# UM-ARM-Lab/pytorch_volumetric

Hardware: AMD Instinct MI355X
Metric: SDF (val+grad) queries/sec (higher is better)
Workload: dtype f32

## Files before the change

pytorch_volumetric_amd/csrc/cached.hip:

```cpp
#include "common.h"
#include "grid_lookup.h"

namespace pvamd {

constexpr int kWavesPerBlock = 16;
constexpr int kTilePoints = 256;
constexpr int64_t kWaveTileMinPoints = 16384;
constexpr int kCqMinWaves = 1;
constexpr int64_t kCqStreamFrom = (int64_t)8 << 20;
constexpr bool kCqBigStNt = true, kCqBigLdNt = true;
constexpr int64_t kCqBlocks = 1024, kCqBigBlocks = 0;

template <bool F64, bool WRITE_OOB, bool LD_NT, bool ST_NT>
__global__ __launch_bounds__(kWavesPerBlock * 64, kCqMinWaves) void cached_query_wave(const pvamd_grid_t g,
                                                                         const float* __restrict__ pts, int64_t P,
                                                                         float* __restrict__ val,
                                                                         float* __restrict__ grad,
                                                                         uint8_t* __restrict__ oob) {
    __shared__ __attribute__((aligned(16))) float lds[kWavesPerBlock][1024];
    const int lane = threadIdx.x & 63, wave = threadIdx.x >> 6;
    float* spf = lds[wave];
    f32x4_alias* sp = reinterpret_cast<f32x4_alias*>(spf);
    const int64_t ntiles = (P + kTilePoints - 1) / kTilePoints;
    const int64_t wstride = (int64_t)gridDim.x * kWavesPerBlock;
    int64_t tile = (int64_t)blockIdx.x * kWavesPerBlock + wave;
    auto first_point = [&](int64_t t) { return t * kTilePoints <= P - kTilePoints ? t * kTilePoints : P - kTilePoints; };
    f32x4 a, b, c;
    auto load3 = [&](int64_t t) {
        const f32x4_u* src = reinterpret_cast<const f32x4_u*>(pts + 3 * first_point(t));
        if (LD_NT) {
            a = __builtin_nontemporal_load(src + lane);
            b = __builtin_nontemporal_load(src + lane + 64);
            c = __builtin_nontemporal_load(src + lane + 128);
        } else {
            a = src[lane];
            b = src[lane + 64];
            c = src[lane + 128];
        }
    };
    if (tile < ntiles) load3(tile);
    for (; tile < ntiles; tile += wstride) {
        sp[lane] = a;
        sp[lane + 64] = b;
        sp[lane + 128] = c;
        const int64_t next = tile + wstride;
        if (next < ntiles) load3(next);
        PVAMD_WAVE_SYNC();
        float px[4], py[4], pz[4];
        const f32x4 q0 = sp[3 * lane], q1 = sp[3 * lane + 1], q2 = sp[3 * lane + 2];
        px[0] = q0.x; py[0] = q0.y; pz[0] = q0.z;
        px[1] = q0.w; py[1] = q1.x; pz[1] = q1.y;
        px[2] = q1.z; py[2] = q1.w; pz[2] = q2.x;
        px[3] = q2.y; py[3] = q2.z; pz[3] = q2.w;
        PVAMD_WAVE_SYNC();
        const int64_t o = first_point(tile);
        float4 r[4];
        bool valid[4];
#pragma unroll
        for (int k = 0; k < 4; ++k) {
            r[k] = cached_lookup<F64, LD_NT>(g, px[k], py[k], pz[k], valid[k]);
        }
        sp[3 * lane] = f32x4{r[0].y, r[0].z, r[0].w, r[1].y};
        sp[3 * lane + 1] = f32x4{r[1].z, r[1].w, r[2].y, r[2].z};
        sp[3 * lane + 2] = f32x4{r[2].w, r[3].y, r[3].z, r[3].w};
        const f32x4 v4 = f32x4{r[0].x, r[1].x, r[2].x, r[3].x};
        if constexpr (WRITE_OOB) {
            const uint32_t m = (valid[0] ? 0u : 1u) | (valid[1] ? 0u : 1u << 8) | (valid[2] ? 0u : 1u << 16) | (valid[3] ? 0u : 1u << 24);
            __builtin_memcpy(oob + o + 4 * lane, &m, 4);
        }
        PVAMD_WAVE_SYNC();
        f32x4_u* vdst = reinterpret_cast<f32x4_u*>(val + o);
        f32x4_u* dst = reinterpret_cast<f32x4_u*>(grad + 3 * o);
        if (ST_NT) {
            __builtin_nontemporal_store(v4, vdst + lane);
            __builtin_nontemporal_store(sp[lane], dst + lane);
            __builtin_nontemporal_store(sp[lane + 64], dst + lane + 64);
            __builtin_nontemporal_store(sp[lane + 128], dst + lane + 128);
        } else {
            vdst[lane] = v4;
            dst[lane] = sp[lane];
            dst[lane + 64] = sp[lane + 64];
            dst[lane + 128] = sp[lane + 128];
        }
        PVAMD_WAVE_SYNC();
    }
}

template <bool F64, bool WRITE_OOB, int PPL, int WAVES>
__global__ __launch_bounds__(WAVES * 64) void cached_query_direct(const pvamd_grid_t g, const float* __restrict__ pts, int64_t P,
                                                                  float* __restrict__ val, float* __restrict__ grad,
                                                                  uint8_t* __restrict__ oob) {
    constexpr int kTile = 64 * PPL;
    const int lane = threadIdx.x & 63, wave = threadIdx.x >> 6;
    const int64_t tile = (int64_t)blockIdx.x * WAVES + wave;
    if (tile * kTile >= P) return;
    const int64_t o = (tile * kTile <= P - kTile ? tile * kTile : P - kTile) + lane;
    float px[PPL], py[PPL], pz[PPL];
#pragma unroll
    for (int k = 0; k < PPL; ++k) {
        const int64_t i = o + 64 * k;
        px[k] = pts[3 * i];
        py[k] = pts[3 * i + 1];
        pz[k] = pts[3 * i + 2];
    }
#pragma unroll
    for (int k = 0; k < PPL; ++k) {
        const int64_t i = o + 64 * k;
        bool valid;
        const float4 r = cached_lookup<F64, false>(g, px[k], py[k], pz[k], valid);
        __builtin_nontemporal_store(r.x, val + i);
        __builtin_nontemporal_store(r.y, grad + 3 * i);
        __builtin_nontemporal_store(r.z, grad + 3 * i + 1);
        __builtin_nontemporal_store(r.w, grad + 3 * i + 2);
        if constexpr (WRITE_OOB) oob[i] = valid ? 0 : 1;
    }
}

enum CqKind {
    kCqScalar = PVAMD_CQ_KERNEL_SCALAR, kCqDirect1 = PVAMD_CQ_KERNEL_DIRECT_1, kCqDirect2 = PVAMD_CQ_KERNEL_DIRECT_2,
    kCqDirect2Wide = PVAMD_CQ_KERNEL_DIRECT_2W, kCqDirect4 = PVAMD_CQ_KERNEL_DIRECT_4, kCqWaveTile = PVAMD_CQ_KERNEL_WAVE_TILE,
    kCqStreaming = PVAMD_CQ_KERNEL_STREAMING
};
static inline CqKind cq_kind(int64_t P) {
    if (P < kWaveTileMinPoints) return kCqScalar;
    if (P <= 160 * 1024) return kCqDirect1;
    if (P <= 896 * 1024) return kCqDirect2;
    if (P <= 1024 * 1024) return kCqDirect2Wide;
    if (P <= 1600 * 1024) return kCqDirect4;
    if (P <= 2304 * 1024) return kCqWaveTile;
    if (P <= kCqStreamFrom) return kCqDirect4;
    return kCqStreaming;
}

template <bool F64>
__global__ __launch_bounds__(256) void cached_query_scalar(const pvamd_grid_t g, const float* __restrict__ pts,
                                                            int64_t first, int64_t P, float* __restrict__ val,
                                                            float* __restrict__ grad, uint8_t* __restrict__ oob) {
    const int64_t stride = (int64_t)gridDim.x * blockDim.x;
    for (int64_t i = first + (int64_t)blockIdx.x * blockDim.x + threadIdx.x; i < P; i += stride) {
        bool valid;
        const float4 r = cached_lookup<F64>(g, pts[3 * i], pts[3 * i + 1], pts[3 * i + 2], valid);
        val[i] = r.x;
        grad[3 * i] = r.y;
        grad[3 * i + 1] = r.z;
        grad[3 * i + 2] = r.w;
        if (oob) oob[i] = valid ? 0 : 1;
    }
}

template <bool F64>
__global__ __launch_bounds__(256) void cached_outside_kernel(const pvamd_grid_t g, const float* __restrict__ pts,
                                                              int64_t P, float level, uint8_t* __restrict__ out) {
    const int64_t stride = (int64_t)gridDim.x * blockDim.x;
    for (int64_t i = (int64_t)blockIdx.x * blockDim.x + threadIdx.x; i < P; i += stride) {
        int flat;
        const bool valid = voxel_flat<F64>(g, pts[3 * i], pts[3 * i + 1], pts[3 * i + 2], flat);
        out[i] = valid ? (uint8_t)(g.vox[4 * (int64_t)flat] > level) : (uint8_t)1;
    }
}

template <bool F64>
__global__ __launch_bounds__(256) void voxel_index_kernel(const pvamd_grid_t g, const float* __restrict__ pts,
                                                           int64_t P, int64_t* __restrict__ out_key,
                                                           int64_t* __restrict__ out_flat,
                                                           uint8_t* __restrict__ out_valid) {
    const int64_t stride = (int64_t)gridDim.x * blockDim.x;
    for (int64_t i = (int64_t)blockIdx.x * blockDim.x + threadIdx.x; i < P; i += stride) {
        long long key[3];
        const bool valid = voxel_key<F64>(g, pts[3 * i], pts[3 * i + 1], pts[3 * i + 2], key);
        if (out_key) {
            out_key[3 * i] = key[0];
            out_key[3 * i + 1] = key[1];
            out_key[3 * i + 2] = key[2];
        }
        if (out_flat) out_flat[i] = (key[0] * g.shape[1] + key[1]) * g.shape[2] + key[2];
        if (out_valid) out_valid[i] = valid ? 1 : 0;
    }
}

__global__ __launch_bounds__(256) void cached_outside_f64_kernel(const pvamd_grid_t g, const double* __restrict__ pts,
                                                                  int64_t P, double level, uint8_t* __restrict__ out) {
    const int64_t stride = (int64_t)gridDim.x * blockDim.x;
    for (int64_t i = (int64_t)blockIdx.x * blockDim.x + threadIdx.x; i < P; i += stride) {
        const double p[3] = {pts[3 * i], pts[3 * i + 1], pts[3 * i + 2]};
        long long key[3];
        const bool valid = voxel_key_f64(g, p, key);
        out[i] = valid ? (uint8_t)(g.vox[4 * (int64_t)clamped_flat(g, key)] > (float)level) : (uint8_t)1;
    }
}

__global__ __launch_bounds__(256) void voxel_index_f64_kernel(const pvamd_grid_t g, const double* __restrict__ pts,
                                                               int64_t P, int64_t* __restrict__ out_key,
                                                               int64_t* __restrict__ out_flat,
                                                               uint8_t* __restrict__ out_valid) {
    const int64_t stride = (int64_t)gridDim.x * blockDim.x;
    for (int64_t i = (int64_t)blockIdx.x * blockDim.x + threadIdx.x; i < P; i += stride) {
        const double p[3] = {pts[3 * i], pts[3 * i + 1], pts[3 * i + 2]};
        long long key[3];
        const bool valid = voxel_key_f64(g, p, key);
        if (out_key) {
            out_key[3 * i] = key[0];
            out_key[3 * i + 1] = key[1];
            out_key[3 * i + 2] = key[2];
        }
        if (out_flat) out_flat[i] = (key[0] * g.shape[1] + key[1]) * g.shape[2] + key[2];
        if (out_valid) out_valid[i] = valid ? 1 : 0;
    }
}

__global__ __launch_bounds__(256) void pack_grid_kernel(const float* __restrict__ val, const float* __restrict__ grad,
                                                         int64_t n, float4* __restrict__ out) {
    const int64_t stride = (int64_t)gridDim.x * blockDim.x;
    for (int64_t i = (int64_t)blockIdx.x * blockDim.x + threadIdx.x; i < n; i += stride) {
        out[i] = make_float4(val[i], grad[3 * i], grad[3 * i + 1], grad[3 * i + 2]);
    }
}

}

using namespace pvamd;

extern "C" int pvamd_pack_grid(const float* val, const float* grad, int64_t n, float* out, void* stream) {
    if (!val || !grad || !out) return PVAMD_E_NULL;
    if (n < 0) return PVAMD_E_SHAPE;
    if (!aligned_to(out, 16)) return PVAMD_E_ALIGN;
    if (n == 0) return 0;
    hipLaunchKernelGGL(pack_grid_kernel, dim3(stream_grid(n, 256)), dim3(256), 0, (hipStream_t)stream, val, grad, n,
                       reinterpret_cast<float4*>(out));
    return (int)hipGetLastError();
}

extern "C" int pvamd_cached_query_kernel(int64_t P) { return (int)cq_kind(P); }

extern "C" int pvamd_cached_query(const pvamd_grid_t* grid, const float* points, int64_t P, float* out_val,
                                  float* out_grad, uint8_t* out_oob, void* stream) {
    if (P < 0) return PVAMD_E_SHAPE;
    if (P == 0) return 0;
    if (!grid || !out_val || !out_grad || !points) return PVAMD_E_NULL;
    if (int e = check_grid(*grid)) return e;
    if (!aligned_to(points, 4) || !aligned_to(out_val, 4) || !aligned_to(out_grad, 4)) return PVAMD_E_ALIGN;
    hipStream_t s = (hipStream_t)stream;
    const bool f64 = grid->index_f64 != 0;
    const CqKind kind = cq_kind(P);
    if (kind == kCqWaveTile || kind == kCqStreaming) {
        const int64_t ntiles = (P + kTilePoints - 1) / kTilePoints;
        const int64_t need = (ntiles + kWavesPerBlock - 1) / kWavesPerBlock;
        const bool big = kind == kCqStreaming;
        const int64_t cap = big ? kCqBigBlocks : kCqBlocks;
        const dim3 grid_dim((unsigned)((cap > 0 && need > cap) ? cap : need)), block(kWavesPerBlock * 64);
#define PVAMD_LAUNCH_CQ(F64_, OOB_)                                                                                      \
    do {                                                                                                                \
        if (big) hipLaunchKernelGGL((cached_query_wave<F64_, OOB_, kCqBigLdNt, kCqBigStNt>), grid_dim, block, 0, s, *grid, points, P, out_val, out_grad, out_oob); \
        else hipLaunchKernelGGL((cached_query_wave<F64_, OOB_, false, true>), grid_dim, block, 0, s, *grid, points, P, out_val, out_grad, out_oob);    \
    } while (0)
        if (f64) {
            if (out_oob) PVAMD_LAUNCH_CQ(true, true);
            else PVAMD_LAUNCH_CQ(true, false);
        } else {
            if (out_oob) PVAMD_LAUNCH_CQ(false, true);
            else PVAMD_LAUNCH_CQ(false, false);
        }
#undef PVAMD_LAUNCH_CQ
    } else if (kind != kCqScalar) {
#define PVAMD_LAUNCH_DIRECT(PPL_, WAVES_)                                                                               \
    do {                                                                                                                \
        const int64_t tiles_ = (P + 64 * PPL_ - 1) / (64 * PPL_);                                                       \
        const dim3 grid_dim((unsigned)((tiles_ + WAVES_ - 1) / WAVES_)), block(WAVES_ * 64);                            \
        if (f64) {                                                                                                      \
            if (out_oob) hipLaunchKernelGGL((cached_query_direct<true, true, PPL_, WAVES_>), grid_dim, block, 0, s, *grid, points, P, out_val, out_grad, out_oob);   \
            else hipLaunchKernelGGL((cached_query_direct<true, false, PPL_, WAVES_>), grid_dim, block, 0, s, *grid, points, P, out_val, out_grad, out_oob);        \
        } else {                                                                                                        \
            if (out_oob) hipLaunchKernelGGL((cached_query_direct<false, true, PPL_, WAVES_>), grid_dim, block, 0, s, *grid, points, P, out_val, out_grad, out_oob);  \
            else hipLaunchKernelGGL((cached_query_direct<false, false, PPL_, WAVES_>), grid_dim, block, 0, s, *grid, points, P, out_val, out_grad, out_oob);       \
        }                                                                                                               \
    } while (0)
        if (kind == kCqDirect1) PVAMD_LAUNCH_DIRECT(1, 8);
        else if (kind == kCqDirect2) PVAMD_LAUNCH_DIRECT(2, 4);
        else if (kind == kCqDirect2Wide) PVAMD_LAUNCH_DIRECT(2, 16);
        else PVAMD_LAUNCH_DIRECT(4, 4);
#undef PVAMD_LAUNCH_DIRECT
    } else {
        const dim3 grid_dim(stream_grid(P, 256)), block(256);
        if (f64) hipLaunchKernelGGL((cached_query_scalar<true>), grid_dim, block, 0, s, *grid, points, (int64_t)0, P, out_val, out_grad, out_oob);
        else hipLaunchKernelGGL((cached_query_scalar<false>), grid_dim, block, 0, s, *grid, points, (int64_t)0, P, out_val, out_grad, out_oob);
    }
    return (int)hipGetLastError();
}

extern "C" int pvamd_cached_outside(const pvamd_grid_t* grid, const float* points, int64_t P, float level,
                                    uint8_t* out, void* stream) {
    if (P < 0) return PVAMD_E_SHAPE;
    if (P == 0) return 0;
    if (!grid || !out || !points) return PVAMD_E_NULL;
    if (int e = check_grid(*grid)) return e;
    const dim3 grid_dim(stream_grid(P, 256)), block(256);
    if (grid->index_f64) hipLaunchKernelGGL((cached_outside_kernel<true>), grid_dim, block, 0, (hipStream_t)stream, *grid, points, P, level, out);
    else hipLaunchKernelGGL((cached_outside_kernel<false>), grid_dim, block, 0, (hipStream_t)stream, *grid, points, P, level, out);
    return (int)hipGetLastError();
}

extern "C" int pvamd_voxel_index(const pvamd_grid_t* grid, const float* points, int64_t P, int64_t* out_key,
                                 int64_t* out_flat, uint8_t* out_valid, void* stream) {
    if (P < 0) return PVAMD_E_SHAPE;
    if (P == 0) return 0;
    if (!grid || !points) return PVAMD_E_NULL;
    if (int e = check_grid(*grid, false)) return e;
    const dim3 grid_dim(stream_grid(P, 256)), block(256);
    if (grid->index_f64) hipLaunchKernelGGL((voxel_index_kernel<true>), grid_dim, block, 0, (hipStream_t)stream, *grid, points, P, out_key, out_flat, out_valid);
    else hipLaunchKernelGGL((voxel_index_kernel<false>), grid_dim, block, 0, (hipStream_t)stream, *grid, points, P, out_key, out_flat, out_valid);
    return (int)hipGetLastError();
}

extern "C" int pvamd_cached_outside_f64(const pvamd_grid_t* grid, const double* points, int64_t P, double level,
                                        uint8_t* out, void* stream) {
    if (P < 0) return PVAMD_E_SHAPE;
    if (P == 0) return 0;
    if (!grid || !out || !points) return PVAMD_E_NULL;
    if (int e = check_grid(*grid)) return e;
    if (!aligned_to(points, 8)) return PVAMD_E_ALIGN;
    hipLaunchKernelGGL(cached_outside_f64_kernel, dim3(stream_grid(P, 256)), dim3(256), 0, (hipStream_t)stream, *grid,
                       points, P, level, out);
    return (int)hipGetLastError();
}

extern "C" int pvamd_voxel_index_f64(const pvamd_grid_t* grid, const double* points, int64_t P, int64_t* out_key,
                                     int64_t* out_flat, uint8_t* out_valid, void* stream) {
    if (P < 0) return PVAMD_E_SHAPE;
    if (P == 0) return 0;
    if (!grid || !points) return PVAMD_E_NULL;
    if (int e = check_grid(*grid, false)) return e;
    if (!aligned_to(points, 8)) return PVAMD_E_ALIGN;
    hipLaunchKernelGGL(voxel_index_f64_kernel, dim3(stream_grid(P, 256)), dim3(256), 0, (hipStream_t)stream, *grid, points,
                       P, out_key, out_flat, out_valid);
    return (int)hipGetLastError();
}
```

pytorch_volumetric_amd/csrc/grid_lookup.h:

```cpp
#pragma once
#include <hip/hip_runtime.h>
#include <stdint.h>
#include "exact_math.h"
#include "../../include/pvamd.h"

namespace pvamd {

#define PVAMD_DEV __device__ __forceinline__

typedef float record_f32x4 __attribute__((ext_vector_type(4)));
typedef const record_f32x4 __attribute__((address_space(1))) * global_record_ptr;
PVAMD_DEV float4 load_record(const float* vox, int flat) {
    const record_f32x4 r = ((global_record_ptr)(uintptr_t)vox)[flat];
    return make_float4(r.x, r.y, r.z, r.w);
}

template <typename T>
PVAMD_DEV T round_by_rule(int rule, T q) {
    if (rule & PVAMD_RULE_ROUND_HALF_AWAY) {
        if constexpr (sizeof(T) == 8) return __builtin_round(q);
        else return __builtin_roundf(q);
    }
    if (rule & PVAMD_RULE_ROUND_FLOOR_HALF) {
        if constexpr (sizeof(T) == 8) return __builtin_floor(q + 0.5);
        else return __builtin_floorf(add_rn(q, 0.5f));
    }
    if constexpr (sizeof(T) == 8) return __builtin_rint(q);
    else return __builtin_rintf(q);
}

PVAMD_DEV bool voxel_index_1d_ruled(const pvamd_grid_t& g, int d, float p, bool f64, long long& k) {
    double kq;
    if (f64) kq = round_by_rule<double>(g.rule, ((double)p - g.dmin[d]) / g.dres[d]);
    else kq = (double)round_by_rule<float>(g.rule, div_rn(sub_rn(p, g.fmin[d]), g.fres[d]));
    k = (long long)kq;
    if (g.rule & PVAMD_RULE_VALID_ON_INDEX) return (kq >= 0.0) && (kq <= (double)(g.shape[d] - 1));
    return f64 ? (g.dmin[d] <= (double)p) && ((double)p <= g.dmax[d]) : (g.fmin[d] <= p) && (p <= g.fmax[d]);
}

template <bool F64>
PVAMD_DEV bool voxel_index_1d(const pvamd_grid_t& g, int d, float p, long long& k) {
    if (__builtin_expect(g.rule != 0, 0)) return voxel_index_1d_ruled(g, d, p, F64, k);
    if constexpr (F64) {
        const double pd = (double)p;
        const bool valid = (g.dmin[d] <= pd) && (pd <= g.dmax[d]);
        k = (long long)__builtin_rint((pd - g.dmin[d]) / g.dres[d]);
        return valid;
    } else {
        const bool valid = (g.fmin[d] <= p) && (p <= g.fmax[d]);
        k = (long long)__builtin_rintf(div_rn(sub_rn(p, g.fmin[d]), g.fres[d]));
        return valid;
    }
}

template <bool F64>
PVAMD_DEV bool voxel_key(const pvamd_grid_t& g, float x, float y, float z, long long key[3]) {
    const bool vx = voxel_index_1d<F64>(g, 0, x, key[0]);
    const bool vy = voxel_index_1d<F64>(g, 1, y, key[1]);
    const bool vz = voxel_index_1d<F64>(g, 2, z, key[2]);
    return vx & vy & vz;
}

template <bool F64>
PVAMD_DEV bool voxel_flat(const pvamd_grid_t& g, float x, float y, float z, int& flat) {
    long long key[3];
    const bool valid = voxel_key<F64>(g, x, y, z, key);
    int kx = (int)key[0], ky = (int)key[1], kz = (int)key[2];
    kx = min(max(kx, 0), g.shape[0] - 1);
    ky = min(max(ky, 0), g.shape[1] - 1);
    kz = min(max(kz, 0), g.shape[2] - 1);
    flat = (kx * g.shape[1] + ky) * g.shape[2] + kz;
    return valid;
}

PVAMD_DEV bool in_range(const pvamd_grid_t& g, float x, float y, float z) {
    return (g.vlo[0] <= x) & (x <= g.vhi[0]) & (g.vlo[1] <= y) & (y <= g.vhi[1]) & (g.vlo[2] <= z) & (z <= g.vhi[2]);
}

PVAMD_DEV uint64_t in_range_mask(const pvamd_grid_t& g, float x, float y, float z) {
    return __builtin_amdgcn_ballot_w64(__builtin_amdgcn_fmed3f(x, g.vlo[0], g.vhi[0]) == x) &
           __builtin_amdgcn_ballot_w64(__builtin_amdgcn_fmed3f(y, g.vlo[1], g.vhi[1]) == y) &
           __builtin_amdgcn_ballot_w64(__builtin_amdgcn_fmed3f(z, g.vlo[2], g.vhi[2]) == z);
}

template <bool F64>
PVAMD_DEV int voxel_index_fast(const pvamd_grid_t& g, int d, float p) {
    const float t = mul_rn(sub_rn(p, g.fmin[d]), g.inv32[d]);
    const float kc = __builtin_rintf(t);
    const float half_dist = sub_rn(0.5f, fabsf(sub_rn(t, kc)));
    if (half_dist > g.err32[d]) return (int)kc;
    long long k;
    voxel_index_1d<F64>(g, d, p, k);
    return (int)k;
}

PVAMD_DEV bool wave_all(bool p) { return __builtin_amdgcn_ballot_w64(p) == __builtin_amdgcn_ballot_w64(true); }
PVAMD_DEV bool wave_any(bool p) { return __builtin_amdgcn_ballot_w64(p) != 0; }

PVAMD_DEV float sqrt_rn_sumsq(float n2) {
    const bool tiny = (unsigned)(__float_as_int(n2) - 1) < (unsigned)(0x0F800000 - 1);
    if (__builtin_expect(wave_any(tiny), 0)) return sqrt_rn(n2);
    float s = __builtin_amdgcn_sqrtf(n2);
    const float s_dn = __int_as_float(__float_as_int(s) - 1), s_up = __int_as_float(__float_as_int(s) + 1);
    const float r_dn = fmaf(-s_dn, s, n2), r_up = fmaf(-s_up, s, n2);
    s = (r_dn <= 0.f) ? s_dn : s;
    s = (r_up > 0.f) ? s_up : s;
    return s;
}

PVAMD_DEV bool estimate_unsure(const pvamd_grid_t& g, const float off[3]) {
    const float worst = __builtin_fmaxf(__builtin_fmaxf(fabsf(off[0]), fabsf(off[1])), fabsf(off[2]));
    return !(sub_rn(0.5f, worst) > g.err32[0]);
}

PVAMD_DEV int voxel_flat_estimate(const pvamd_grid_t& g, float x, float y, float z, bool& unsure) {
    const float p[3] = {x, y, z};
    int k[3];
    float off[3];
#pragma unroll
    for (int d = 0; d < 3; ++d) {
        const float t = mul_rn(sub_rn(p[d], g.fmin[d]), g.inv32[d]);
        const float kc = __builtin_rintf(t);
        off[d] = sub_rn(t, kc);
        k[d] = (int)kc;
    }
    unsure |= estimate_unsure(g, off);
    const unsigned flat = (unsigned)((k[0] * g.shape[1] + k[1]) * g.shape[2] + k[2]);
    const unsigned last = (unsigned)(g.shape[0] * g.shape[1] * g.shape[2] - 1);
    return (int)(flat < last ? flat : last);
}

PVAMD_DEV int voxel_flat_in_range_fused(const pvamd_grid_t& g, float x, float y, float z) {
    const float p[3] = {x, y, z};
    int k[3];
    float off[3];
#pragma unroll
    for (int d = 0; d < 3; ++d) {
        const float t = mul_rn(sub_rn(p[d], g.fmin[d]), g.inv32[d]);
        const float kc = __builtin_rintf(t);
        off[d] = sub_rn(t, kc);
        k[d] = (int)kc;
    }
    const bool unsure = estimate_unsure(g, off);
    if (__builtin_expect(wave_any(unsure), 0)) {
        if (unsure) {
#pragma unroll 1
            for (int d = 0; d < 3; ++d) {
                long long kd;
                if (g.index_f64) voxel_index_1d<true>(g, d, p[d], kd);
                else voxel_index_1d<false>(g, d, p[d], kd);
                k[d] = (int)kd;
            }
        }
    }
    const unsigned flat = (unsigned)((k[0] * g.shape[1] + k[1]) * g.shape[2] + k[2]);
    const unsigned last = (unsigned)(g.shape[0] * g.shape[1] * g.shape[2] - 1);
    return (int)(flat < last ? flat : last);
}

template <bool F64>
PVAMD_DEV int voxel_flat_in_range(const pvamd_grid_t& g, float x, float y, float z) {
    int kx = voxel_index_fast<F64>(g, 0, x), ky = voxel_index_fast<F64>(g, 1, y), kz = voxel_index_fast<F64>(g, 2, z);
    kx = min(max(kx, 0), g.shape[0] - 1);
    ky = min(max(ky, 0), g.shape[1] - 1);
    kz = min(max(kz, 0), g.shape[2] - 1);
    return (kx * g.shape[1] + ky) * g.shape[2] + kz;
}

PVAMD_DEV float bounding_box_vector(const pvamd_grid_t& g, float x, float y, float z, float t[3]) {
    const float p[3] = {x, y, z};
#pragma unroll
    for (int d = 0; d < 3; ++d) {
        float lo = sub_rn(g.bb_min[d], p[d]);
        const bool lo_active = lo > 0.f;
        lo = lo_active ? lo : 0.f;
        float hi = sub_rn(p[d], g.bb_max[d]);
        hi = (hi > 0.f) ? hi : 0.f;
        const float s = add_rn(lo, hi);
        t[d] = lo_active ? -s : s;
    }
    return sqrt_rn(fmaf(t[2], t[2], fmaf(t[1], t[1], mul_rn(t[0], t[0]))));
}

PVAMD_DEV float4 bounding_box_sdf(const pvamd_grid_t& g, float x, float y, float z) {
    float t[3];
    const float n = bounding_box_vector(g, x, y, z, t);
    return make_float4(n, div_rn(t[0], n), div_rn(t[1], n), div_rn(t[2], n));
}

template <bool F64, bool STREAMING = false>
PVAMD_DEV float4 cached_lookup(const pvamd_grid_t& g, float x, float y, float z, bool& valid) {
    if constexpr (STREAMING) {
        valid = in_range(g, x, y, z);
        if (valid) {
            return reinterpret_cast<const float4*>(g.vox)[voxel_flat_in_range<F64>(g, x, y, z)];
        }
        if (g.oob_mode == PVAMD_OOB_BOUNDING_BOX) {
            return bounding_box_sdf(g, x, y, z);
        }
        return make_float4(0.f, 0.f, 0.f, 0.f);
    } else {
        valid = (__builtin_amdgcn_fmed3f(x, g.vlo[0], g.vhi[0]) == x) & (__builtin_amdgcn_fmed3f(y, g.vlo[1], g.vhi[1]) == y) &
                (__builtin_amdgcn_fmed3f(z, g.vlo[2], g.vhi[2]) == z);
        if (valid) return reinterpret_cast<const float4*>(g.vox)[voxel_flat_in_range_fused(g, x, y, z)];
        if (g.oob_mode == PVAMD_OOB_BOUNDING_BOX) {
            const float ta = __builtin_amdgcn_fmed3f(sub_rn(x, g.bb_min[0]), sub_rn(x, g.bb_max[0]), 0.f);
            const float tb = __builtin_amdgcn_fmed3f(sub_rn(y, g.bb_min[1]), sub_rn(y, g.bb_max[1]), 0.f);
            const float tc = __builtin_amdgcn_fmed3f(sub_rn(z, g.bb_min[2]), sub_rn(z, g.bb_max[2]), 0.f);
            const float n = sqrt_rn_sumsq(fmaf(tc, tc, fmaf(tb, tb, mul_rn(ta, ta))));
            return make_float4(n, div_rn(ta, n), div_rn(tb, n), div_rn(tc, n));
        }
        return make_float4(0.f, 0.f, 0.f, 0.f);
    }
}

PVAMD_DEV bool voxel_key_f64(const pvamd_grid_t& g, const double p[3], long long key[3]) {
    bool valid = true;
#pragma unroll
    for (int d = 0; d < 3; ++d) {
        const double kq = round_by_rule<double>(g.rule, (p[d] - g.dmin[d]) / g.dres[d]);
        key[d] = (long long)kq;
        if (__builtin_expect(g.rule & PVAMD_RULE_VALID_ON_INDEX, 0)) valid &= (kq >= 0.0) && (kq <= (double)(g.shape[d] - 1));
        else valid &= (g.dmin[d] <= p[d]) && (p[d] <= g.dmax[d]);
    }
    return valid;
}

PVAMD_DEV int clamped_flat(const pvamd_grid_t& g, const long long key[3]) {
    const int kx = min(max((int)key[0], 0), g.shape[0] - 1);
    const int ky = min(max((int)key[1], 0), g.shape[1] - 1);
    const int kz = min(max((int)key[2], 0), g.shape[2] - 1);
    return (kx * g.shape[1] + ky) * g.shape[2] + kz;
}

PVAMD_DEV float affine_row(float m0, float m1, float m2, float m3, float px, float py, float pz) {
    return add_rn(fmaf(m2, pz, fmaf(m1, py, mul_rn(m0, px))), m3);
}

template <typename T> struct LeafOps;

template <> struct LeafOps<float> {
    static PVAMD_DEV void xform(const float* M, const float p[3], float x[3]) {
        x[0] = affine_row(M[0], M[1], M[2], M[3], p[0], p[1], p[2]);
        x[1] = affine_row(M[4], M[5], M[6], M[7], p[0], p[1], p[2]);
        x[2] = affine_row(M[8], M[9], M[10], M[11], p[0], p[1], p[2]);
    }
    static PVAMD_DEV bool inside(const pvamd_grid_t& g, const float x[3]) { return in_range(g, x[0], x[1], x[2]); }
    static PVAMD_DEV void record_grad(const pvamd_grid_t& g, const float x[3], float gr[3]) {
        int flat;
        if (g.index_f64) voxel_flat<true>(g, x[0], x[1], x[2], flat);
        else voxel_flat<false>(g, x[0], x[1], x[2], flat);
        const float4 r = load_record(g.vox, flat);
        gr[0] = r.y; gr[1] = r.z; gr[2] = r.w;
    }
    static PVAMD_DEV float box(const pvamd_grid_t& g, const float x[3], float t[3]) {
        return bounding_box_vector(g, x[0], x[1], x[2], t);
    }
    static PVAMD_DEV float div(float a, float b) { return div_rn(a, b); }
};

template <> struct LeafOps<double> {
    static PVAMD_DEV void xform(const double* M, const double p[3], double x[3]) {
#pragma unroll
        for (int r = 0; r < 3; ++r)
            x[r] = __builtin_fma(M[4 * r + 2], p[2], __builtin_fma(M[4 * r + 1], p[1], M[4 * r] * p[0])) + M[4 * r + 3];
    }
    static PVAMD_DEV bool inside(const pvamd_grid_t& g, const double x[3]) {
        long long key[3];
        return voxel_key_f64(g, x, key);
    }
    static PVAMD_DEV void record_grad(const pvamd_grid_t& g, const double x[3], double gr[3]) {
        long long key[3];
        voxel_key_f64(g, x, key);
        const float4 r = load_record(g.vox, clamped_flat(g, key));
        gr[0] = (double)r.y; gr[1] = (double)r.z; gr[2] = (double)r.w;
    }
    static PVAMD_DEV double box(const pvamd_grid_t& g, const double x[3], double t[3]) {
#pragma unroll
        for (int d = 0; d < 3; ++d) {
            double lo = g.dbb_min[d] - x[d];
            const bool lo_active = lo > 0.0;
            lo = lo_active ? lo : 0.0;
            double hi = x[d] - g.dbb_max[d];
            hi = (hi > 0.0) ? hi : 0.0;
            const double s = lo + hi;
            t[d] = lo_active ? -s : s;
        }
        return __builtin_sqrt(__builtin_fma(t[2], t[2], __builtin_fma(t[1], t[1], t[0] * t[0])));
    }
    static PVAMD_DEV double div(double a, double b) { return a / b; }
};

}
```

Baseline: 203.0 billion.

## Batch voxel record gathers in direct kernel and compute bbox fallback branch-free

The direct cached-query kernel now computes validity and flat indices for all PPL points per lane first, with a wave-uniform slow path for uncertain indices. It then issues all record loads back to back, computes the bounding-box fallback unconditionally, and selects results per point. This is meant to expose memory-level parallelism across the gathered loads instead of serialising lookup, load and store per point, at the cost of extra ALU work and registers for the unconditional bbox math. The early return for out-of-range tiles is removed, and the wave-tile size threshold is lowered slightly.

```diff
diff --git a/pytorch_volumetric_amd/csrc/cached.hip b/pytorch_volumetric_amd/csrc/cached.hip
--- a/pytorch_volumetric_amd/csrc/cached.hip
+++ b/pytorch_volumetric_amd/csrc/cached.hip
@@ -90,10 +90,10 @@
 __global__ __launch_bounds__(WAVES * 64) void cached_query_direct(const pvamd_grid_t g, const float* __restrict__ pts, int64_t P,
                                                                   float* __restrict__ val, float* __restrict__ grad,
                                                                   uint8_t* __restrict__ oob) {
+    static_assert(PPL >= 1 && PPL <= 4, "the gathered records live in four named variables");
     constexpr int kTile = 64 * PPL;
     const int lane = threadIdx.x & 63, wave = threadIdx.x >> 6;
     const int64_t tile = (int64_t)blockIdx.x * WAVES + wave;
-    if (tile * kTile >= P) return;
     const int64_t o = (tile * kTile <= P - kTile ? tile * kTile : P - kTile) + lane;
     float px[PPL], py[PPL], pz[PPL];
 #pragma unroll
@@ -103,16 +103,48 @@
         py[k] = pts[3 * i + 1];
         pz[k] = pts[3 * i + 2];
     }
+    bool valid[PPL], unsure[PPL];
+    int flat[PPL];
+    bool any_unsure = false;
+#pragma unroll
+    for (int k = 0; k < PPL; ++k) {
+        valid[k] = in_range_med3(g, px[k], py[k], pz[k]);
+        unsure[k] = false;
+        flat[k] = voxel_flat_estimate(g, px[k], py[k], pz[k], unsure[k]);
+        unsure[k] &= valid[k];
+        any_unsure |= unsure[k];
+    }
+    if (__builtin_expect(wave_any(any_unsure), 0)) {
+#pragma unroll
+        for (int k = 0; k < PPL; ++k) {
+            if (unsure[k]) voxel_flat<F64>(g, px[k], py[k], pz[k], flat[k]);
+        }
+    }
+    record_f32x4 rec_a, rec_b, rec_c, rec_d;
+    if (valid[0]) rec_a = load_record_bits(g.vox, flat[0]);
+    if constexpr (PPL > 1) { if (valid[1]) rec_b = load_record_bits(g.vox, flat[1]); }
+    if constexpr (PPL > 2) { if (valid[2]) rec_c = load_record_bits(g.vox, flat[2]); }
+    if constexpr (PPL > 3) { if (valid[3]) rec_d = load_record_bits(g.vox, flat[3]); }
+    const bool bbox = g.oob_mode == PVAMD_OOB_BOUNDING_BOX;
+    float4 ob[PPL];
+#pragma unroll
+    for (int k = 0; k < PPL; ++k) {
+        ob[k] = bbox ? bounding_box_record(g, px[k], py[k], pz[k]) : make_float4(0.f, 0.f, 0.f, 0.f);
+    }
 #pragma unroll
     for (int k = 0; k < PPL; ++k) {
         const int64_t i = o + 64 * k;
-        bool valid;
-        const float4 r = cached_lookup<F64, false>(g, px[k], py[k], pz[k], valid);
-        __builtin_nontemporal_store(r.x, val + i);
-        __builtin_nontemporal_store(r.y, grad + 3 * i);
-        __builtin_nontemporal_store(r.z, grad + 3 * i + 1);
-        __builtin_nontemporal_store(r.w, grad + 3 * i + 2);
-        if constexpr (WRITE_OOB) oob[i] = valid ? 0 : 1;
+        const bool v = valid[k];
+        const record_f32x4& rec = k == 0 ? rec_a : k == 1 ? rec_b : k == 2 ? rec_c : rec_d;
+        const uint32_t r0 = v ? __float_as_uint(rec.x) : __float_as_uint(ob[k].x);
+        const uint32_t r1 = v ? __float_as_uint(rec.y) : __float_as_uint(ob[k].y);
+        const uint32_t r2 = v ? __float_as_uint(rec.z) : __float_as_uint(ob[k].z);
+        const uint32_t r3 = v ? __float_as_uint(rec.w) : __float_as_uint(ob[k].w);
+        __builtin_nontemporal_store(__uint_as_float(r0), val + i);
+        __builtin_nontemporal_store(__uint_as_float(r1), grad + 3 * i);
+        __builtin_nontemporal_store(__uint_as_float(r2), grad + 3 * i + 1);
+        __builtin_nontemporal_store(__uint_as_float(r3), grad + 3 * i + 2);
+        if constexpr (WRITE_OOB) oob[i] = v ? 0 : 1;
     }
 }
 
@@ -127,7 +159,7 @@
     if (P <= 896 * 1024) return kCqDirect2;
     if (P <= 1024 * 1024) return kCqDirect2Wide;
     if (P <= 1600 * 1024) return kCqDirect4;
-    if (P <= 2304 * 1024) return kCqWaveTile;
+    if (P <= 2048 * 1024) return kCqWaveTile;
     if (P <= kCqStreamFrom) return kCqDirect4;
     return kCqStreaming;
 }
diff --git a/pytorch_volumetric_amd/csrc/grid_lookup.h b/pytorch_volumetric_amd/csrc/grid_lookup.h
--- a/pytorch_volumetric_amd/csrc/grid_lookup.h
+++ b/pytorch_volumetric_amd/csrc/grid_lookup.h
@@ -10,8 +10,9 @@
 
 typedef float record_f32x4 __attribute__((ext_vector_type(4)));
 typedef const record_f32x4 __attribute__((address_space(1))) * global_record_ptr;
+PVAMD_DEV record_f32x4 load_record_bits(const float* vox, int flat) { return ((global_record_ptr)(uintptr_t)vox)[flat]; }
 PVAMD_DEV float4 load_record(const float* vox, int flat) {
-    const record_f32x4 r = ((global_record_ptr)(uintptr_t)vox)[flat];
+    const record_f32x4 r = load_record_bits(vox, flat);
     return make_float4(r.x, r.y, r.z, r.w);
 }
 
@@ -186,6 +187,19 @@
     float t[3];
     const float n = bounding_box_vector(g, x, y, z, t);
     return make_float4(n, div_rn(t[0], n), div_rn(t[1], n), div_rn(t[2], n));
+}
+
+PVAMD_DEV float4 bounding_box_record(const pvamd_grid_t& g, float x, float y, float z) {
+    const float ta = __builtin_amdgcn_fmed3f(sub_rn(x, g.bb_min[0]), sub_rn(x, g.bb_max[0]), 0.f);
+    const float tb = __builtin_amdgcn_fmed3f(sub_rn(y, g.bb_min[1]), sub_rn(y, g.bb_max[1]), 0.f);
+    const float tc = __builtin_amdgcn_fmed3f(sub_rn(z, g.bb_min[2]), sub_rn(z, g.bb_max[2]), 0.f);
+    const float n = sqrt_rn_sumsq(fmaf(tc, tc, fmaf(tb, tb, mul_rn(ta, ta))));
+    return make_float4(n, div_rn(ta, n), div_rn(tb, n), div_rn(tc, n));
+}
+
+PVAMD_DEV bool in_range_med3(const pvamd_grid_t& g, float x, float y, float z) {
+    return (__builtin_amdgcn_fmed3f(x, g.vlo[0], g.vhi[0]) == x) & (__builtin_amdgcn_fmed3f(y, g.vlo[1], g.vhi[1]) == y) &
+           (__builtin_amdgcn_fmed3f(z, g.vlo[2], g.vhi[2]) == z);
 }
 
 template <bool F64, bool STREAMING = false>
@@ -200,16 +214,9 @@
         }
         return make_float4(0.f, 0.f, 0.f, 0.f);
     } else {
-        valid = (__builtin_amdgcn_fmed3f(x, g.vlo[0], g.vhi[0]) == x) & (__builtin_amdgcn_fmed3f(y, g.vlo[1], g.vhi[1]) == y) &
-                (__builtin_amdgcn_fmed3f(z, g.vlo[2], g.vhi[2]) == z);
+        valid = in_range_med3(g, x, y, z);
         if (valid) return reinterpret_cast<const float4*>(g.vox)[voxel_flat_in_range_fused(g, x, y, z)];
-        if (g.oob_mode == PVAMD_OOB_BOUNDING_BOX) {
-            const float ta = __builtin_amdgcn_fmed3f(sub_rn(x, g.bb_min[0]), sub_rn(x, g.bb_max[0]), 0.f);
-            const float tb = __builtin_amdgcn_fmed3f(sub_rn(y, g.bb_min[1]), sub_rn(y, g.bb_max[1]), 0.f);
-            const float tc = __builtin_amdgcn_fmed3f(sub_rn(z, g.bb_min[2]), sub_rn(z, g.bb_max[2]), 0.f);
-            const float n = sqrt_rn_sumsq(fmaf(tc, tc, fmaf(tb, tb, mul_rn(ta, ta))));
-            return make_float4(n, div_rn(ta, n), div_rn(tb, n), div_rn(tc, n));
-        }
+        if (g.oob_mode == PVAMD_OOB_BOUNDING_BOX) return bounding_box_record(g, x, y, z);
         return make_float4(0.f, 0.f, 0.f, 0.f);
     }
 }
```

Result: faster. 211.9 billion, median of 6 (+4.4%).
